# Quaternijkon/hnsw-ivf

Hardware: AMD Instinct MI355X
Metric: queries/sec @ recall@10, IVF4096 d=128 nq=10k nprobe=32; 1/2/4/8 GPUs (higher is better)
Workload: dtype f32; 1 GPU; IVF4096,Flat; d=128, nb=1000000, vectors_per_gpu=1000000, nq_per_gpu=10000, nprobe=32, k=10, global_batch=10000, parallelism=single, grid_point=False

## Files before the change

hnsw-ivf_amd/csrc/bf3.h:

```cpp
#pragma once

#include <hip/hip_runtime.h>

#include <cstdint>

#include "wave_select.h"

namespace faiss_amd {
namespace kern {

typedef __bf16 bf16x8 __attribute__((ext_vector_type(8)));
typedef float floatx16 __attribute__((ext_vector_type(16)));

constexpr int BQ = 64;
constexpr int FQ = 128;
constexpr int BV = 64;
constexpr int BDM = 128;

__device__ __forceinline__ uint32_t med3_u32(uint32_t a, uint32_t b, uint32_t c) {
    uint32_t r;
    asm("v_med3_u32 %0, %1, %2, %3" : "=v"(r) : "v"(a), "v"(b), "v"(c));
    return r;
}

// ... 29 lines not shown
__device__ __forceinline__ float key_decode_lo(uint32_t key, uint32_t lowmask) {
    return L2 ? __uint_as_float(key & ~lowmask) : unordered_f32(key & ~lowmask);
}
template <bool L2>
__device__ __forceinline__ float key_decode_hi(uint32_t key, uint32_t lowmask) {
    return L2 ? __uint_as_float(key | lowmask) : unordered_f32(key | lowmask);
}

__device__ __forceinline__ uint32_t fold_key_bits(float acc) { return __float_as_uint(acc); }
__device__ __forceinline__ void mfma_read_guard() {
    __builtin_amdgcn_sched_barrier(0);
    asm volatile("s_nop 15" ::: "memory");
    __builtin_amdgcn_sched_barrier(0);
}
__device__ __forceinline__ float fold_decode_lo(uint32_t key, uint32_t lowmask) {
    return fmaxf(-2.f * __uint_as_float(key & ~lowmask), 0.f);
}
__device__ __forceinline__ float fold_decode_hi(uint32_t key, uint32_t lowmask) {
    return fmaxf(-2.f * __uint_as_float(key | lowmask), 0.f);
}
template <bool L2>
__device__ __forceinline__ float ivf_decode_lo(uint32_t key, uint32_t lowmask, bool fold) {
    return (L2 && fold) ? fold_decode_lo(key, lowmask) : key_decode_lo<L2>(key, lowmask);
}
template <bool L2>
__device__ __forceinline__ float ivf_decode_hi(uint32_t key, uint32_t lowmask, bool fold) {
    return (L2 && fold) ? fold_decode_hi(key, lowmask) : key_decode_hi<L2>(key, lowmask);
}
__device__ __forceinline__ void split3_bf16(float v, __bf16& h, __bf16& m, __bf16& l) {
    h = (__bf16)v;
    const float r1 = v - (float)h;
    m = (__bf16)r1;
    l = (__bf16)(r1 - (float)m);
}

__device__ __forceinline__ void split8(const float (&v)[8], bf16x8& h, bf16x8& l) {
#pragma unroll
    for (int j = 0; j < 8; j++) {
        const __bf16 hb = (__bf16)v[j];
        h[j] = hb;
        l[j] = (__bf16)(v[j] - (float)hb);
    }
}

template <int NS>
__device__ __forceinline__ void query_raw_load(const float* __restrict__ x, int ldx, int d, int qr,
                                               int lh, float4 (&raw)[2 * NS]) {
    const float* xr = x + (int64_t)(qr < 0 ? 0 : qr) * ldx;
    const int d4 = (d + 3) & ~3;
#pragma unroll
    for (int s = 0; s < NS; s++)
#pragma unroll
        for (int u = 0; u < 2; u++) {
            const int kk = 16 * s + 8 * lh + 4 * u;
            raw[2 * s + u] = *(const float4*)(xr + min(kk, d4 - 4));
        }
}
template <int NS>
__device__ __forceinline__ void query_frags_from_raw(const float4 (&raw)[2 * NS], int d, int lh,
                                                     bf16x8 (&bh)[NS], bf16x8 (&bl)[NS],
                                                     float& xn) {
    xn = 0.f;
#pragma unroll
    for (int s = 0; s < NS; s++) {
        float v[8] = {raw[2 * s].x,     raw[2 * s].y,     raw[2 * s].z,     raw[2 * s].w,
                      raw[2 * s + 1].x, raw[2 * s + 1].y, raw[2 * s + 1].z, raw[2 * s + 1].w};
#pragma unroll
        for (int j = 0; j < 8; j++) v[j] = 16 * s + 8 * lh + j < d ? v[j] : 0.f;
        split8(v, bh[s], bl[s]);
#pragma unroll
        for (int j = 0; j < 8; j++) xn = fmaf(v[j], v[j], xn);
    }
    xn += __shfl_xor(xn, 32);
}
template <int NS>
__device__ __forceinline__ void load_query_frags(const float* __restrict__ x, int ldx, int d,
                                                 int qr, int lh, bf16x8 (&bh)[NS],
                                                 bf16x8 (&bl)[NS], float& xn) {
    float4 raw[2 * NS];
    query_raw_load<NS>(x, ldx, d, qr, lh, raw);
    query_frags_from_raw<NS>(raw, d, lh, bh, bl, xn);
}

template <int NS>
__device__ __forceinline__ void load_query_image(const uint8_t* __restrict__ qimg,
                                                 const float* __restrict__ qxn, int qr, int lh,
                                                 bf16x8 (&bh)[NS], bf16x8 (&bl)[NS], float& xn) {
    const int q = qr < 0 ? 0 : qr;
    const uint8_t* row = qimg + (int64_t)q * (64 * NS) + 16 * lh;
#pragma unroll
    for (int s = 0; s < NS; s++) {
        bh[s] = *(const bf16x8*)(row + 32 * s);
        bl[s] = *(const bf16x8*)(row + 32 * NS + 32 * s);
    }
    xn = qxn ? qxn[q] : 0.f;
}

template <int NS>
__device__ __forceinline__ floatx16 bf3_block(const uint8_t* arow, const bf16x8 (&bh)[NS],
                                              const bf16x8 (&bl)[NS]) {
    constexpr int DB = 16 * NS;
    bf16x8 ah[NS], al[NS];
#pragma unroll
    for (int s = 0; s < NS; s++) {
        ah[s] = *(const bf16x8*)(arow + 32 * s);
        al[s] = *(const bf16x8*)(arow + 2 * DB + 32 * s);
    }
    floatx16 acc;
#pragma unroll
    for (int r = 0; r < 16; r++) acc[r] = 0.f;
#pragma unroll
    for (int s = 0; s < NS; s++) {
        acc = __builtin_amdgcn_mfma_f32_32x32x16_bf16(al[s], bh[s], acc, 0, 0, 0);
        acc = __builtin_amdgcn_mfma_f32_32x32x16_bf16(ah[s], bl[s], acc, 0, 0, 0);
        acc = __builtin_amdgcn_mfma_f32_32x32x16_bf16(ah[s], bh[s], acc, 0, 0, 0);
    }
    return acc;
}

template <int NS>
__device__ __forceinline__ floatx16 bf2_block(const uint8_t* arow, const bf16x8 (&bh)[NS],
                                              const bf16x8 (&bl)[NS]) {
    bf16x8 ah[NS];
#pragma unroll
    for (int s = 0; s < NS; s++) ah[s] = *(const bf16x8*)(arow + 32 * s);
    floatx16 acc;
#pragma unroll
    for (int r = 0; r < 16; r++) acc[r] = 0.f;
#pragma unroll
    for (int s = 0; s < NS; s++) {
        acc = __builtin_amdgcn_mfma_f32_32x32x16_bf16(ah[s], bl[s], acc, 0, 0, 0);
        acc = __builtin_amdgcn_mfma_f32_32x32x16_bf16(ah[s], bh[s], acc, 0, 0, 0);
    }
    return acc;
}

__device__ __forceinline__ uint32_t cdiv_dev(uint32_t a, uint32_t b) { return (a + b - 1) / b; }

__device__ __forceinline__ uint32_t ivf_key_row(uint32_t key, uint32_t lowmask, int slot) {
    const uint32_t ord = key & lowmask;
    const uint32_t r = ord & 15u;
    return (ord >> 4) * BV + 32 * (slot >> 1) + 4 * (slot & 1) + 8 * (r >> 2) + (r & 3);
}

__device__ __forceinline__ int ivf_stream_row(int e, int slot) {
    const int r = e & 15;
    return (e >> 4) * BV + 32 * (slot >> 1) + 4 * (slot & 1) + 8 * (r >> 2) + (r & 3);
}

inline int bf3_db(int d) { return (d + 31) / 32 * 32; }

}
}
```

hnsw-ivf_amd/csrc/core.cpp:

```cpp
#include <algorithm>
#include <cfloat>
#include <cmath>
#include <cstdlib>
#include <cstring>
#include <thread>

#include "../../include/faiss_amd.h"
#include "kernels.h"

namespace faiss_amd {
namespace kern {
void mask_columns(float* D, int64_t nx, int64_t ny, int64_t ldD, const uint8_t* mask, float v,
                  hipStream_t s);
}

IndexIVFStats indexIVF_stats;
HNSWStats hnsw_stats;
HNSWRowStats hnsw_row_stats;

std::mutex InterruptCallback::lock;
std::unique_ptr<InterruptCallback> InterruptCallback::instance;

void InterruptCallback::clear_instance() { instance.reset(); }

// ... 222 lines not shown
            kern::row_resnorm_bf16(d_xb_.as<float>(), ntotal, d, l, s_tile_.as<float>(), s);
            kern::array_max(s_tile_.as<float>(), ntotal, d_cnmax_.as<float>() + 1, s);
            d_cst_.reserve(kern::coarse_stream_image_bytes(ntotal, d));
            const char* fenv = getenv("FAISS_AMD_COARSE_FOLD");
            cfold_ = (metric_type == METRIC_L2 && !(fenv && !strcmp(fenv, "0"))) ? 1 : 0;
            kern::coarse_stream_image(d_xb_.as<float>(), ntotal, d, l, d_norms_.as<float>(),
                                      d_cst_.ptr, s, cfold_);
        }
    }
    HIP_CHECK(hipStreamSynchronize(s));
    dirty_ = false;
}

const float* IndexFlat::device_vectors() const {
    sync_device();
    return d_xb_.as<float>();
}
size_t IndexFlat::query_image_size(idx_t n) const {
    return kern::query_image_bytes(n, d) + sizeof(float) * n;
}
const float* IndexFlat::device_norms() const {
    sync_device();
    return d_norms_.as<float>();
}

template <class OutIdx>
bool IndexFlat::knn_device(idx_t n, const float* x, int ldx, int k, float* distances,
                           OutIdx* labels, hipStream_t s, void* qimg_out, idx_t batch_n) const {
    FAISS_THROW_IF_NOT_FMT(k >= 1, "k = %d must be >= 1", k);
    sync_device();
    std::lock_guard<std::recursive_mutex> g(mu_);
    order_.enter(s);
    const bool direct = (batch_n >= 0 ? batch_n : n) < 20;
    const bool img = knn_impl<OutIdx>(n, x, ldx, k, distances, labels, s, qimg_out, direct);
    order_.leave(s);
    return img;
}

template <class OutIdx>
bool IndexFlat::knn_impl(idx_t n, const float* x, int ldx, int k, float* distances,
                         OutIdx* labels, hipStream_t s, void* qimg_out, bool direct) const {
    const int l = ld();
    const int metric_l2 = metric_type == METRIC_L2;
    const bool ip_chunked = !metric_l2 && ntotal > ((idx_t)1 << 20);
    FAISS_THROW_IF_NOT_MSG(!(ip_chunked && k <= kern::kMaxK && sizeof(OutIdx) == 4),
                           "coarse quantizer larger than 2^20 centroids");
    if (k > kern::kMaxK || ip_chunked) {
        if (metric_l2) {
            s_xn_.reserve(sizeof(float) * std::max<idx_t>(n, 1));
            kern::row_norms(x, n, d, ldx, s_xn_.as<float>(), s);
        }
        const idx_t ny = std::max<idx_t>(ntotal, 1);
        const idx_t qc = std::max<idx_t>(1, std::min<idx_t>(n, ((idx_t)1 << 28) / ny));
        s_tile_.reserve(sizeof(float) * qc * ny);
        ScopedKernelTimer tm(&ktimes, "flat_distance+select_exact", 2.0 * n * ntotal * d, s);
        for (idx_t q0 = 0; q0 < n; q0 += qc) {
            const idx_t nq = std::min(qc, n - q0);
            if (ntotal > 0 && direct)
                kern::direct_distances(x + q0 * ldx, nq, ldx, d_xb_.as<float>(), ntotal, l, d,
                                       metric_l2, s_tile_.as<float>(), ntotal, s);
            else if (ntotal > 0)
                kern::pairwise_distances(x + q0 * ldx, nq, ldx,
                                         metric_l2 ? s_xn_.as<float>() + q0 : nullptr,
                                         d_xb_.as<float>(), ntotal, l, d_norms_.as<float>(), l,
                                         metric_l2, s_tile_.as<float>(), ntotal, s);
            kern::select_rows_exact<OutIdx>(s_tile_.as<float>(), nq, ntotal, ntotal, k,
                                            metric_l2, 0, distances + q0 * k, labels + q0 * k, k,
                                            s, &s_sel_);
        }
        return false;
    }
    constexpr bool i32 = sizeof(OutIdx) == 4;
    int32_t* o32 = i32 ? (int32_t*)labels : nullptr;
    int64_t* o64 = i32 ? nullptr : (int64_t*)labels;
    const idx_t ny = ntotal;
    s_xn_.reserve(sizeof(float) * std::max<idx_t>(n, 1));
    const char* cenv = getenv("FAISS_AMD_COARSE");
    const kern::CoarsePlan plan =
            (cenv && !strcmp(cenv, "f32")) || ny > (1 << 20) || d_cbf_.ptr == nullptr || direct
                    ? kern::CoarsePlan{}
                    : kern::coarse_bf3_plan(n, (int)ny, d, k);
    if (plan.ok) {
        const bool qi = d_cst_.ptr != nullptr && ldx % 4 == 0;
        void* qimg = nullptr;
        if (qi) {
            const size_t ib = kern::query_image_bytes(n, d);
            if (!qimg_out) s_qimg_.reserve(ib + sizeof(float) * n);
            qimg = qimg_out ? qimg_out : s_qimg_.ptr;
            ScopedKernelTimer tq(&ktimes, "query_prep", 0.0, s);
            kern::query_prep(x, n, ldx, d, s_xn_.as<float>(), qimg, (float*)((uint8_t*)qimg + ib),
                             s);
        } else {
            kern::row_norms(x, n, d, ldx, s_xn_.as<float>(), s);
        }
        const size_t per_q = (size_t)plan.entries * 4 + plan.nsplit * 16;
        const idx_t qchunk = std::max<idx_t>(64, (idx_t)(((size_t)256 << 20) / per_q) / 64 * 64);
        const idx_t qc = std::min<idx_t>(qchunk, n);
        s_cand_i_.reserve(sizeof(uint32_t) * qc * plan.entries);
        s_tile_.reserve(sizeof(float) * qc * plan.nsplit * 4);
        for (idx_t q0 = 0; q0 < n; q0 += qc) {
            const idx_t nq = std::min(qc, n - q0);
            kern::coarse_bf3_knn(plan, x + q0 * ldx, nq, ldx, s_xn_.as<float>() + q0,
                                 d_xb_.as<float>(), l, d_cbf_.ptr, d_norms_.as<float>(),
                                 d_cnmax_.as<float>(), (int)ny, d, k, metric_l2,
                                 s_cand_i_.as<uint32_t>(), s_tile_.as<float>(), distances + q0 * k,
                                 o32 ? o32 + q0 * k : nullptr, o64 ? o64 + q0 * k : nullptr, s,
                                 d_cst_.ptr,
                                 qi ? (const uint8_t*)qimg + q0 * kern::query_image_bytes(1, d)
                                    : nullptr,
                                 &ktimes, cfold_);
        }
        return qi && qimg_out;
    }
    if (metric_l2) kern::row_norms(x, n, d, ldx, s_xn_.as<float>(), s);
    const idx_t Yc = std::min<idx_t>(std::max<idx_t>(ny, 1), 1 << 20);
    const idx_t nyc = (idx_t)cdiv(std::max<idx_t>(ny, 1), Yc);
    FAISS_THROW_IF_NOT_MSG(!(i32 && nyc > 1), "coarse quantizer larger than 2^20 centroids");
    const size_t tile_budget = (size_t)256 << 20;
    idx_t qchunk = std::max<idx_t>(128, (idx_t)(tile_budget / (sizeof(float) * Yc)) / 128 * 128);
    qchunk = std::min<idx_t>(qchunk, n);
    s_tile_.reserve(sizeof(float) * qchunk * Yc);
    if (nyc > 1) {
        s_cand_d_.reserve(sizeof(float) * nyc * qchunk * k);
        s_cand_i_.reserve(sizeof(idx_t) * nyc * qchunk * k);
    }
    double flops = 2.0 * (double)n * (double)ny * (double)d;
    ScopedKernelTimer tm(&ktimes, "flat_distance+select", flops, s);
    for (idx_t q0 = 0; q0 < n; q0 += qchunk) {
        const idx_t nq = std::min(qchunk, n - q0);
        const float* xq = x + q0 * ldx;
        const float* xn = s_xn_.as<float>() + q0;
        if (nyc == 1) {
            if (ny > 0 && direct)
                kern::direct_distances(xq, nq, ldx, d_xb_.as<float>(), ny, l, d, metric_l2,
                                       s_tile_.as<float>(), ny, s);
            else if (ny > 0)
                kern::pairwise_distances(xq, nq, ldx, xn, d_xb_.as<float>(), ny, l,
                                         d_norms_.as<float>(), l, metric_l2,
                                         s_tile_.as<float>(), ny, s);
            kern::select_rows(s_tile_.as<float>(), nq, ny, ny, k, metric_l2, 0,
                              distances + q0 * k, o32 ? o32 + q0 * k : nullptr,
                              o64 ? o64 + q0 * k : nullptr, k, s);
            if (!metric_l2 && ny > 0)
                kern::select_fix_ip(s_tile_.as<float>(), nq, ny, ny, k, distances + q0 * k,
                                    o32 ? o32 + q0 * k : nullptr, o64 ? o64 + q0 * k : nullptr,
                                    k, s);
        } else {
            for (idx_t c = 0; c < nyc; c++) {
                const idx_t y0 = c * Yc, nyy = std::min(Yc, ny - y0);
                if (direct)
                    kern::direct_distances(xq, nq, ldx, d_xb_.as<float>() + y0 * l, nyy, l, d,
                                           metric_l2, s_tile_.as<float>(), nyy, s);
                else
                    kern::pairwise_distances(xq, nq, ldx, xn, d_xb_.as<float>() + y0 * l, nyy,
                                             l, d_norms_.as<float>() + y0, l, metric_l2,
                                             s_tile_.as<float>(), nyy, s);
                kern::select_rows(s_tile_.as<float>(), nq, nyy, nyy, k, metric_l2, y0,
                                  s_cand_d_.as<float>() + c * nq * k, nullptr,
                                  s_cand_i_.as<int64_t>() + c * nq * k, k, s);
            }
            kern::merge_rows(s_cand_d_.as<float>(), s_cand_i_.as<int64_t>(), nq,
                             (int)((nyc << 16) | k), k, metric_l2, distances + q0 * k,
                             o64 + q0 * k, s);
        }
    }
    return false;
}

void IndexFlat::search_device(idx_t n, const float* x, int ldx, idx_t k, float* distances,
                              idx_t* labels, const SearchParameters* params,
                              hipStream_t s) const {
    DeviceGuard g(device);
    if (params && params->sel) {
        search_selected(n, x, ldx, k, distances, labels, params->sel, s);
        return;
    }
    knn_device<idx_t>(n, x, ldx, (int)k, distances, labels, s);
}

const idx_t* IndexFlat::device_row_ids(hipStream_t s) const {
    std::lock_guard<std::recursive_mutex> g(mu_);
    if (selids_n_ != ntotal) {
        std::vector<idx_t> iota((size_t)ntotal);
        for (idx_t i = 0; i < ntotal; i++) iota[(size_t)i] = i;
        s_selids_.reserve(sizeof(idx_t) * ntotal);
        HIP_CHECK(hipMemcpyAsync(s_selids_.ptr, iota.data(), sizeof(idx_t) * ntotal,
                                 hipMemcpyHostToDevice, s));
        HIP_CHECK(hipStreamSynchronize(s));
        selids_n_ = ntotal;
    }
    return s_selids_.as<idx_t>();
}

// ... 366 lines not shown
```

hnsw-ivf_amd/csrc/kernels.h:

```cpp
#pragma once

#include <hip/hip_runtime.h>
#include <algorithm>
#include <cstdint>

#include "common.h"

namespace faiss_amd {
namespace kern {

constexpr int kMaxK = 64;
constexpr int kMaxNprobeFilter = 2048;
constexpr int kMaxKExact = 2048;

void row_norms(const float* x, int64_t n, int d, int ld, float* out, hipStream_t s);

void pairwise_distances(const float* x, int64_t nx, int ldx, const float* xn,
                        const float* y, int64_t ny, int ldy, const float* yn, int dp,
                        int metric_l2, float* D, int64_t ldD, hipStream_t s);

void direct_distances(const float* x, int64_t nx, int ldx, const float* y, int64_t ny, int ldy,
                      int d, int metric_l2, float* D, int64_t ldD, hipStream_t s);

struct CoarsePlan {
    bool ok = false;
    int nsplit = 0, split_len = 0, kt = 0, obits = 0, entries = 0;
};
CoarsePlan coarse_bf3_plan(int64_t n, int nlist, int d, int k);
void coarse_bf3_knn(const CoarsePlan& p, const float* x, int64_t n, int ldx, const float* xnorm,
                    const float* cent, int ldc, const void* cbf, const float* cnorm,
                    const float* cnmax, int nlist, int d, int k, int metric_l2, uint32_t* keys,
                    float* pbs, float* D, int32_t* I32, int64_t* I64, hipStream_t s,
                    const void* cst = nullptr, const void* qimg = nullptr,
                    KernelTimes* kt = nullptr,
                    int fold = 0);
void query_prep(const float* x, int64_t n, int ldx, int d, float* ref_norms, void* qimg,
                float* qxn, hipStream_t s);
inline size_t query_image_bytes(int64_t n, int d) {
    return (size_t)std::max<int64_t>(n, 1) * 4 * ((d + 31) / 32 * 32);
}
void coarse_stream_image(const float* codes, int64_t rows, int d, int ldc, const float* norms,
                         void* out, hipStream_t s, int fold = 0);
size_t coarse_stream_image_bytes(int64_t rows, int d);
void array_max(const float* a, int64_t n, float* out, hipStream_t s);

void select_rows(const float* D, int64_t nx, int64_t ny, int64_t ldD, int k, int metric_l2,
                 int64_t col0, float* out_d, int32_t* out_i32, int64_t* out_i64,
                 int64_t ldo, hipStream_t s);

void select_fix_ip(const float* D, int64_t nx, int64_t ny, int64_t ldD, int k, float* out_d,
                   int32_t* out_i32, int64_t* out_i64, int64_t ldo, hipStream_t s);

void merge_rows(const float* cand_d, const int64_t* cand_i, int64_t n, int nin_x_kin, int k,
                int metric_l2, float* out_d, int64_t* out_i, hipStream_t s);

void merge_rows_general(const float* cand_d, const int64_t* cand_i, int64_t n, int nshard,
                        int kin, int k, int metric_l2, float* out_d, int64_t* out_i,
                        hipStream_t s);

void translate_labels(int64_t* labels, int64_t n, int64_t offset, hipStream_t s);

struct alignas(16) ProbeRec {
    float pb[4];
    float mmax;
    uint32_t off;
    uint32_t len;
    uint32_t pad;
};

struct alignas(16) ItemDesc {
    uint32_t l, nq, len, off;
};

struct IVFBuckets {
    uint32_t* counts;
    uint32_t* bucket_off;
    uint32_t* item_off;
    uint32_t* cursor;
    uint32_t* entries;
    uint32_t* item_list = nullptr;
    uint32_t* item_ctr = nullptr;
    uint32_t* scan_tmp = nullptr;
    uint32_t* ticket = nullptr;
    const uint32_t* perm = nullptr;
    ItemDesc* item_desc = nullptr;
    uint32_t* item_entries = nullptr;
    uint32_t* mark_keys = nullptr;
    ProbeRec* mark_recs = nullptr;
    int mark_ke = 0;
    uint32_t* counts_next = nullptr;
    const uint32_t* lim = nullptr;
    const uint8_t* sel = nullptr;
};
void probe_limits(const int32_t* assign, int64_t n, int nprobe, const uint32_t* list_len,
                  int nlist, int64_t max_codes, int32_t* assign_out, uint32_t* lim,
                  hipStream_t s);
void ivf_bucket(const int32_t* assign, int64_t n, int nprobe, const uint32_t* list_len,
                const uint32_t* list_off, int nlist, int QT, IVFBuckets b, hipStream_t s);
void ivf_flat_rerank(const uint32_t* keys, const ProbeRec* recs, const float* x, int ldx,
                     const float* codes, int ldc, const int64_t* ids, int d, int64_t n,
                     int nprobe, int KE, int obits, int k, int metric_l2, const uint8_t* sel,
                     uint32_t* stats, float* D, int64_t* I, KernelTimes* kt, hipStream_t s,
                     unsigned long long* qdone, int fold);
struct PQArgs {
    const float* pq_cent = nullptr;
    const float* cent = nullptr;
    int ldcent = 0;
    const float* cdis = nullptr;
    const uint8_t* codes = nullptr;
    int cs = 0;
    int M = 0;
    int table1 = 0;
};
struct RerankSel {
    const uint8_t* sel = nullptr;
};
bool ivfpq_mfma_eligible(int d, int M, int k, int nprobe);
double ivfpq_mfma_coef(int d, int M);
// ... 238 lines not shown
```

hnsw-ivf_amd/csrc/kernels_coarse.hip:

```cpp
#include <hip/hip_runtime.h>

#include <algorithm>
#include <cfloat>
#include <cstdio>
#include <cstdlib>
#include <cstring>
#include <type_traits>
#include <vector>

#include "bf3.h"
#include "common.h"
#include "exact_select.h"
#include "kernels.h"
#include "ref_arith.h"
#include "wave_select.h"

namespace faiss_amd {
namespace kern {

__device__ __forceinline__ float ip_seq(const float* __restrict__ a, const float* __restrict__ b,
                                        int d) {
    float acc = 0.f;
    int j = 0;
    for (; j + 32 <= d; j += 32) {
// ... 59 lines not shown
#pragma unroll
        for (int s = 0; s < PF; s++) {
            const int e = t + 256 * s;
            const int r = e / RU, c = e - r * RU;
            pf[s] = make_uint4(0u, 0u, 0u, 0u);
            if (e < BV * RU && r < nvn)
                pf[s] = *(const uint4*)(cbf + (int64_t)(c0 + v0n + r) * (2 * DB) + 8 * c);
        }
        if (t < BV / 4) {
            const int r = 4 * t;
            float v[4];
#pragma unroll
            for (int c = 0; c < 4; c++)
                v[c] = r + c < nvn ? (L2 ? cn[v0n + r + c] : 0.f) : WS_INF;
            pn = make_float4(v[0], v[1], v[2], v[3]);
        }
    };
    auto stash = [&](int buf) {
        uint8_t* T = tiles + buf * BV * CSB;
#pragma unroll
        for (int s = 0; s < PF; s++) {
            const int e = t + 256 * s;
            const int r = e / RU, c = e - r * RU;
            if (e < BV * RU) *(uint4*)(T + r * CSB + 16 * c) = pf[s];
        }
        if (t < BV / 4) *(float4*)(&ynt[buf][4 * t]) = pn;
    };
    fetch(0);
    stash(0);
    if (BV < len) fetch(BV);
    __syncthreads();

    ThreadQueue32<KT> tq;
    tq.init();
    const uint32_t lowmask = (1u << obits) - 1u;
    for (int v0 = 0, tile = 0; v0 < len; v0 += BV, tile++) {
        const int buf = tile & 1;
        if (v0 + BV < len) {
            stash(buf ^ 1);
            if (v0 + 2 * BV < len) fetch(v0 + 2 * BV);
        }
        float4 yq[4];
#pragma unroll
        for (int g = 0; g < 4; g++) yq[g] = *(const float4*)(&ynt[buf][32 * bi + 4 * lh + 8 * g]);
        const uint8_t* arow = tiles + buf * BV * CSB + (32 * bi + li) * CSB + 16 * lh;
        const floatx16 acc = Y3 ? bf3_block<NS>(arow, bh, bl) : bf2_block<NS>(arow, bh, bl);
        const uint32_t ordbase = (uint32_t)tile << 4;
#pragma unroll
        for (int r = 0; r < 16; r++) {
            const int g = r >> 2, c = r & 3;
            const float yv = c == 0 ? yq[g].x : c == 1 ? yq[g].y : c == 2 ? yq[g].z : yq[g].w;
            const float a = L2 ? fmaf(-2.f, acc[r], xn + yv) : yv - acc[r];
            tq.push(key_encode<L2>(a, lowmask, ordbase | (uint32_t)r));
        }
        __syncthreads();
    }
    if (q < n) {
        const float M = coarse_margin(xn, cnmax_p, coef, Y3);
        const int E1 = 4 * KT;
        uint32_t* ko = keys + (q * nsplit + sp) * E1 + slot * KT;
#pragma unroll
        for (int i = 0; i < KT; i++) {
            const uint32_t key = tq.q[i];
            const uint32_t row = ivf_key_row(key, lowmask, slot);
            ko[i] = (key != 0xffffffffu && row < (uint32_t)len) ? key : 0xffffffffu;
        }
        const uint32_t last = tq.q[KT - 1];
        float bnd = WS_INF;
        if (last != 0xffffffffu && ivf_key_row(last, lowmask, slot) < (uint32_t)len)
            bnd = key_decode_lo<L2>(last, lowmask);
        pbs[(q * nsplit + sp) * 4 + slot] = bnd < WS_INF ? bnd - M : WS_INF;
    }
}

template <int N>
__device__ __forceinline__ void cwait_vmcnt() {
    static_assert(N >= 0 && N < 64, "vmcnt range");
    __builtin_amdgcn_s_waitcnt((N & 15) | (7 << 4) | (15 << 8) | ((N >> 4) << 14));
}

template <bool L2, int KT, int NS, bool FOLD = false>
__global__ __launch_bounds__(256, NS <= 6 && KT <= 8 ? 3 : 2) void k_coarse_stream(
        const float* __restrict__ x, int ldx, int64_t n, int d, const uint8_t* __restrict__ cst,
        const float* __restrict__ xnorm, int nlist, int nsplit, int split_len, int nqb,
        float coef, const float* __restrict__ cnmax_p, int obits, uint32_t* __restrict__ keys,
        float* __restrict__ pbs, unsigned long long* __restrict__ trace,
        const uint8_t* __restrict__ qimg) {
    unsigned long long* tr = (trace && threadIdx.x == 0) ? trace + 160ull * blockIdx.x : nullptr;
    if (tr) tr[0] = __builtin_amdgcn_s_memtime();
    constexpr int DB = 16 * NS;
    constexpr int SR = 4 * DB + 16;
    constexpr int TB = BV * SR;
    static_assert(TB % 1024 == 0, "tile = whole 1 KB glds blocks");
    constexpr int NG = TB / 1024;
    constexpr int G0 = (NG + 3) / 4;
    constexpr int G3 = NG / 4;
    __shared__ __attribute__((aligned(16))) uint8_t tiles[2 * TB];
    const int t = threadIdx.x, lane = t & 63, w = t >> 6;
    const int li = lane & 31, lh = lane >> 5;
    int sp, qb;
    if ((nsplit & 7) == 0) {
        const int xcd = blockIdx.x & 7, m = blockIdx.x >> 3;
        sp = 8 * (m / nqb) + xcd;
        qb = m % nqb;
    } else {
        sp = blockIdx.x / nqb;
        qb = blockIdx.x % nqb;
    }
    const int c0 = sp * split_len;
    const int len = min(split_len, nlist - c0);
    const int ntile = (len + BV - 1) / BV;
    const int qloc = 32 * w + li;
    const int64_t q = (int64_t)qb * 128 + qloc;
    const bool active = (int64_t)qb * 128 + 32 * w < n;

    auto issue = [&](int j, int b) {
        const uint8_t* src = cst + ((int64_t)c0 + (int64_t)j * BV) * SR + 16 * lane;
        uint8_t* dst = tiles + b * TB;
#pragma unroll
        for (int g = 0; g < G0; g++) {
            const int blk = w + 4 * g;
            if (g < G3 || blk < NG)
                __builtin_amdgcn_global_load_lds(
                        (const void*)(src + blk * 1024),
                        (__attribute__((address_space(3))) void*)(dst + blk * 1024), 16, 0, 0);
        }
    };
    issue(0, 0);
    bf16x8 bh[NS], bl[NS];
    float xn_approx;
    if (active) {
        if (qimg)
            load_query_image<NS>(qimg, nullptr, q < n ? (int)q : -1, lh, bh, bl, xn_approx);
        else
            load_query_frags<NS>(x, ldx, d, q < n ? (int)q : -1, lh, bh, bl, xn_approx);
    }
    const float xn = (active && q < n) ? xnorm[q] : 0.f;
    if (tr) tr[1] = __builtin_amdgcn_s_memtime();
    static_assert(!FOLD || L2, "fold: L2 only");
    bf16x8 bq;
    if constexpr (FOLD) {
        __bf16 h, m, lo;
        split3_bf16(-0.5f * xn, h, m, lo);
        const __bf16 one = (__bf16)1.f, zero = (__bf16)0.f;
        bq[0] = lh ? zero : one;
        bq[1] = lh ? zero : one;
        bq[2] = lh ? zero : one;
        bq[3] = lh ? zero : h;
        bq[4] = lh ? zero : m;
        bq[5] = lh ? zero : lo;
        bq[6] = zero;
        bq[7] = zero;
    }

    ThreadQueue32<KT> tq[2];
    tq[0].init();
    tq[1].init();
    const uint32_t lowmask = (1u << obits) - 1u;
    auto norms = [&](const uint8_t* T, int bi, float (&nv)[16]) {
        const uint8_t* nrow = T + (32 * bi + 4 * lh) * SR + 4 * DB;
#pragma unroll
        for (int r = 0; r < 16; r++) nv[r] = *(const float*)(nrow + (8 * (r >> 2) + (r & 3)) * SR);
    };
    auto push1 = [&](ThreadQueue32<KT>& pq, float accr, float yv0, uint32_t ord) {
        if constexpr (FOLD) {
            pq.push(key_insert(fold_key_bits(accr), lowmask, ord));
            return;
        }
        const float yv = L2 ? yv0 : (yv0 < WS_INF ? 0.f : WS_INF);
        const float a = L2 ? fmaf(-2.f, accr, xn + yv) : yv - accr;
        pq.push(key_insert(key_bits<L2>(a), lowmask, ord));
    };
    auto mfma_push = [&](const uint8_t* T, int bi, const floatx16& pacc, const float (&pn)[16],
                         const uint8_t* pnT, uint32_t pord, ThreadQueue32<KT>& pq) {
        const uint8_t* arow = T + (32 * bi + li) * SR + 16 * lh;
        bf16x8 ah[NS], al[NS];
#pragma unroll
        for (int s2 = 0; s2 < NS; s2++) {
            ah[s2] = *(const bf16x8*)(arow + 32 * s2);
            al[s2] = *(const bf16x8*)(arow + 2 * DB + 32 * s2);
        }
        floatx16 acc;
#pragma unroll
        for (int r = 0; r < 16; r++) acc[r] = 0.f;
#pragma unroll
        for (int s2 = 0; s2 < NS; s2++) {
            acc = __builtin_amdgcn_mfma_f32_32x32x16_bf16(al[s2], bh[s2], acc, 0, 0, 0);
            acc = __builtin_amdgcn_mfma_f32_32x32x16_bf16(ah[s2], bl[s2], acc, 0, 0, 0);
            acc = __builtin_amdgcn_mfma_f32_32x32x16_bf16(ah[s2], bh[s2], acc, 0, 0, 0);
            if (FOLD && s2 == 0) mfma_read_guard();
#pragma unroll
            for (int r = 16 * s2 / NS; r < 16 * (s2 + 1) / NS; r++)
                push1(pq, pacc[r],
                      FOLD ? 0.f
                           : pnT ? *(const float*)(pnT + (8 * (r >> 2) + (r & 3)) * SR) : pn[r],
                      pord | (uint32_t)r);
        }
        if constexpr (FOLD) {
            const bf16x8 ab = *(const bf16x8*)(T + (32 * bi + li) * SR + (lh ? 0 : 4 * DB));
            acc = __builtin_amdgcn_mfma_f32_32x32x16_bf16(ab, bq, acc, 0, 0, 0);
        }
        return acc;
    };
    floatx16 acc0, acc1;
    float n1[16];
    cwait_vmcnt<0>();
    __builtin_amdgcn_s_barrier();
    if (ntile > 1) issue(1, 1);
    if (active) {
        acc0 = bf3_block<NS>(tiles + (0 * SR) + li * SR + 16 * lh, bh, bl);
        if constexpr (FOLD) {
            const bf16x8 ab = *(const bf16x8*)(tiles + li * SR + (lh ? 0 : 4 * DB));
            acc0 = __builtin_amdgcn_mfma_f32_32x32x16_bf16(ab, bq, acc0, 0, 0, 0);
        }
    }
    int b = 0;
    for (int j = 0; j < ntile; j++) {
        const uint8_t* T = tiles + b * TB;
        const uint32_t ordbase = (uint32_t)j << 4;
        if (active) {
// ... 462 lines not shown
        trace[8 * q + 3] = t_u;
        trace[8 * q + 4] = t_c;
        trace[8 * q + 5] = t_e;
        trace[8 * q + 7] = t_f;
    }
    if (stats && valid && lane == 0) {
        atomicAdd(&stats[0], (uint32_t)min(ns, CR_CAP));
        atomicAdd(&stats[1], (uint32_t)__popcll(fmask));
        atomicAdd(&stats[2], st.overflow ? 1u : 0u);
        atomicAdd(&stats[3], done ? 0u : 1u);
        atomicAdd(&stats[4], relayed ? 1u : 0u);
    }
}

__global__ void k_array_max(const float* __restrict__ a, int64_t n, float* __restrict__ out) {
    __shared__ float red[16];
    float m = 0.f;
    for (int64_t i = threadIdx.x; i < n; i += blockDim.x) {
        const float v = a[i];
        m = v < WS_INF ? fmaxf(m, v) : WS_INF;
    }
#pragma unroll
    for (int s = 32; s > 0; s >>= 1) m = fmaxf(m, __shfl_xor(m, s));
    if ((threadIdx.x & 63) == 0) red[threadIdx.x >> 6] = m;
    __syncthreads();
    if (threadIdx.x == 0) {
        float r = 0.f;
        for (int i = 0; i < (int)(blockDim.x >> 6); i++) r = fmaxf(r, red[i]);
        *out = r;
    }
}

CoarsePlan coarse_bf3_plan(int64_t n, int nlist, int d, int k) {
    CoarsePlan p{};
    if (n < 20 || nlist <= 0 || k < 1 || k > kMaxK || bf3_db(d) > BDM)
        return p;
    int ncu = 256, dev = 0;
    if (hipGetDevice(&dev) != hipSuccess ||
        hipDeviceGetAttribute(&ncu, hipDeviceAttributeMultiprocessorCount, dev) != hipSuccess ||
        ncu <= 0)
        ncu = 256;
    (void)hipGetLastError();
    const int64_t nqb = (int64_t)cdiv((size_t)n, 128);

    const bool big_image = coarse_stream_image_bytes(nlist, d) > ((size_t)4 << 20);
    int nsplit = 0, kt = 0, split_len = 0;
    double best = 0.0;
    const char* nsenv = getenv("FAISS_AMD_COARSE_NSPLIT");
    const int ns_force = nsenv ? atoi(nsenv) : 0;
    for (int ns = 1; ns <= std::min(16, std::max(1, nlist / BV)); ns++) {
        if (ns_force > 0 && ns != ns_force) continue;
        if (k > 16 * ns) continue;
        const double lam = (double)k / (4.0 * ns);
        if (lam > 4.0) continue;
        const int kt1 = lam <= 0.25 ? 4 : lam <= 2.0 ? 8 : 16;
        const int sl = (int)roundup(cdiv((size_t)nlist, (size_t)ns), BV);
        const int nsp = (int)cdiv((size_t)nlist, (size_t)sl);
        if ((size_t)sl > ((size_t)BV << 10)) continue;
        const int64_t slots = (bf3_db(d) <= 96 && kt1 <= 8 ? 3 : 2) * (int64_t)ncu;
        const int64_t rounds = (int64_t)cdiv((size_t)(nqb * nsp), (size_t)slots);
        double cost = (double)rounds * (double)cdiv((size_t)sl, BV) * (kt1 + 12);
        if (big_image && nsp % 8 != 0) cost *= 1.15;
        if (nsplit == 0 || cost < best) {
            best = cost;
            nsplit = nsp;
            kt = kt1;
            split_len = sl;
        }
    }
    if (nsplit == 0) return p;
    const int tiles = (int)cdiv((size_t)split_len, BV);
    int b = 0;
    while ((1 << b) < tiles) b++;
    if (4 + b > 14) return p;
    p.ok = true;
    p.nsplit = nsplit;
    p.split_len = split_len;
    p.kt = kt;
    p.obits = 4 + b;
    p.entries = nsplit * 4 * kt;
    return p;
}

void coarse_bf3_knn(const CoarsePlan& p, const float* x, int64_t n, int ldx, const float* xnorm,
                    const float* cent, int ldc, const void* cbf, const float* cnorm,
                    const float* cnmax, int nlist, int d, int k, int metric_l2, uint32_t* keys,
                    float* pbs, float* D, int32_t* I32, int64_t* I64, hipStream_t s,
                    const void* cst, const void* qimg, KernelTimes* kt, int fold) {
    if (n <= 0) return;
    FAISS_THROW_IF_NOT(p.ok);
    static uint32_t* stats = nullptr;
    const bool dbg = getenv("FAISS_AMD_IVF_STATS") != nullptr;
    if (dbg && !stats) HIP_CHECK(hipMalloc(&stats, 32));
    if (dbg) HIP_CHECK(hipMemsetAsync(stats, 0, 32, s));
    FAISS_THROW_IF_NOT(ldx % 4 == 0 && ldc % 4 == 0);
    const int NS = bf3_db(d) / 16;
    const char* prec = getenv("FAISS_AMD_COARSE_PREC");
    const bool y3 = !(prec && !strcmp(prec, "bf16x2"));
    const char* cenv = getenv("FAISS_AMD_COARSE");
    const bool stream = cst && y3 && !(cenv && !strcmp(cenv, "staged"));
    const bool fk = stream && fold != 0 && metric_l2;
    const float coef = (float)(fk ? ivf_bf3f_coef(d) : y3 ? ivf_bf3_coef(d) : ivf_bf2_coef(d));
    static unsigned long long* ctrace_buf = nullptr;
    static int64_t ctrace_n = 0;
    const char* ctr = getenv("FAISS_AMD_COARSE_TRACE");
    unsigned long long* ctrace = nullptr;
    const int64_t nqb = (int64_t)cdiv((size_t)n, stream ? 128 : BQ);
    const int64_t grid = nqb * p.nsplit;
    FAISS_THROW_IF_NOT(grid < (1ll << 31));
    if (ctr && stream) {
        if (ctrace_n < grid) {
            if (ctrace_buf) HIP_CHECK(hipFree(ctrace_buf));
            HIP_CHECK(hipMalloc(&ctrace_buf, 160 * 8 * grid));
            ctrace_n = grid;
        }
        HIP_CHECK(hipMemsetAsync(ctrace_buf, 0, 160 * 8 * grid, s));
        ctrace = ctrace_buf;
    }
#define LAUNCH_NS(L2V, KTV, NSV)                                                              \
    do {                                                                                      \
        if (stream)                                                                           \
            (fk ? k_coarse_stream<L2V, KTV, NSV, L2V> : k_coarse_stream<L2V, KTV, NSV, false>) \
                    <<<kgrid(grid, 256), dim3(256), 0, s>>>(                              \
                    x, ldx, n, d, (const uint8_t*)cst, xnorm, nlist, p.nsplit, p.split_len,   \
                    (int)nqb, coef, cnmax, p.obits, keys, pbs, ctrace,                        \
                    (const uint8_t*)qimg);                                                    \
        else if (y3)                                                                          \
            k_coarse_bf3_filter<L2V, KTV, NSV, true><<<kgrid(grid, 256), dim3(256), 0, s>>>( \
                    x, ldx, n, d, (const __bf16*)cbf, cnorm, xnorm, nlist, p.nsplit,          \
                    p.split_len, coef, cnmax, p.obits, keys, pbs);                            \
        else                                                                                  \
            k_coarse_bf3_filter<L2V, KTV, NSV, false><<<kgrid(grid, 256), dim3(256), 0, s>>>( \
                    x, ldx, n, d, (const __bf16*)cbf, cnorm, xnorm, nlist, p.nsplit,          \
                    p.split_len, coef, cnmax, p.obits, keys, pbs);                            \
    } while (0)
#define LAUNCH_A(L2V, KTV)                     \
    do {                                       \
        if (NS == 2) LAUNCH_NS(L2V, KTV, 2);   \
        else if (NS == 4) LAUNCH_NS(L2V, KTV, 4); \
        else if (NS == 6) LAUNCH_NS(L2V, KTV, 6); \
        else LAUNCH_NS(L2V, KTV, 8);           \
    } while (0)
#define DISPATCH(L2V)                      \
    do {                                   \
        if (p.kt == 4) LAUNCH_A(L2V, 4);   \
        else if (p.kt == 8) LAUNCH_A(L2V, 8); \
        else LAUNCH_A(L2V, 16);            \
    } while (0)
    {
        ScopedKernelTimer tm(kt, "coarse_filter", 0.0, s);
        if (metric_l2) DISPATCH(true);
        else DISPATCH(false);
    }
#undef DISPATCH
#undef LAUNCH_A
#undef LAUNCH_NS
    HIP_LAUNCH_CHECK();
    if (ctrace) {
        std::vector<unsigned long long> h(160 * grid);
        HIP_CHECK(hipMemcpyAsync(h.data(), ctrace, 160 * 8 * grid, hipMemcpyDeviceToHost, s));
        HIP_CHECK(hipStreamSynchronize(s));
        if (FILE* f = fopen(ctr, "wb")) {
            fwrite(h.data(), 8, h.size(), f);
            fclose(f);
        }
    }
    const int E = p.entries;
    const int V = E <= 64 ? 1 : E <= 128 ? 2 : E <= 256 ? 4 : E <= 512 ? 8 : 16;
    FAISS_THROW_IF_NOT(E <= 1024 && V <= p.kt);
#define LAUNCH_R(L2V, OT, OUT, VV)                                                              \
    k_coarse_rerank<L2V, OT, VV><<<kgrid(n, 64), dim3(64), 0, s>>>(                       \
            keys, pbs, x, ldx, xnorm, cent, ldc, cnorm, cnmax, coef, y3 ? 1 : 0, n, d, nlist,  \
            p.nsplit,                                                                           \
            p.split_len, p.kt, p.obits, k, D, OUT, st_ptr, crtrace, fk ? 1 : 0)
#define LAUNCH_RV(L2V, OT, OUT)                  \
    do {                                         \
        if (V == 1) LAUNCH_R(L2V, OT, OUT, 1);   \
        else if (V == 2) LAUNCH_R(L2V, OT, OUT, 2); \
        else if (V == 4) LAUNCH_R(L2V, OT, OUT, 4); \
        else if (V == 8) LAUNCH_R(L2V, OT, OUT, 8); \
        else LAUNCH_R(L2V, OT, OUT, 16);         \
    } while (0)
    uint32_t* const st_ptr = dbg ? stats : nullptr;
    static unsigned long long* crtrace_buf = nullptr;
    static int64_t crtrace_n = 0;
    const char* crt = getenv("FAISS_AMD_CRERANK_TRACE");
    unsigned long long* crtrace = nullptr;
    if (crt) {
        if (crtrace_n < n) {
            if (crtrace_buf) HIP_CHECK(hipFree(crtrace_buf));
            HIP_CHECK(hipMalloc(&crtrace_buf, 64 * n));
            crtrace_n = n;
        }
        HIP_CHECK(hipMemsetAsync(crtrace_buf, 0, 64 * n, s));
        crtrace = crtrace_buf;
    }
    {
        ScopedKernelTimer tm(kt, "coarse_rerank", 0.0, s);
        if (metric_l2) {
            if (I32) LAUNCH_RV(true, int32_t, I32);
            else LAUNCH_RV(true, int64_t, I64);
        } else {
            if (I32) LAUNCH_RV(false, int32_t, I32);
            else LAUNCH_RV(false, int64_t, I64);
        }
    }
#undef LAUNCH_RV
#undef LAUNCH_R
    if (crtrace) {
// ... 27 lines not shown
```

Measured before the change: 40.01 million queries/s.

## Fuse query prep into streaming coarse kernel, writing query image and norms in-kernel

Result: no change. 40.37 million queries/s (median of 6 runs) (+0.9%).

```diff
diff --git a/hnsw-ivf_amd/csrc/bf3.h b/hnsw-ivf_amd/csrc/bf3.h
--- a/hnsw-ivf_amd/csrc/bf3.h
+++ b/hnsw-ivf_amd/csrc/bf3.h
@@ -135,6 +135,57 @@
     query_frags_from_raw<NS>(raw, d, lh, bh, bl, xn);
 }
 
+__device__ __forceinline__ void half_swap(float p, float q, float& a, float& b) {
+    const auto r = __builtin_amdgcn_permlane32_swap(__float_as_uint(p), __float_as_uint(q), false,
+                                                    false);
+    a = __uint_as_float(r[0]);
+    b = __uint_as_float(r[1]);
+}
+
+template <int NS>
+__device__ __forceinline__ void load_query_frags_norm(const float* __restrict__ x, int ldx, int d,
+                                                      int qr, int lh, bf16x8 (&bh)[NS],
+                                                      bf16x8 (&bl)[NS], float& xn, float& rn) {
+    float4 raw[2 * NS];
+    query_raw_load<NS>(x, ldx, d, qr, lh, raw);
+    const int n8 = d & ~7;
+    float c0 = 0.f, c1 = 0.f, c2 = 0.f, c3 = 0.f;
+#pragma unroll
+    for (int s = 0; s < NS; s++) {
+        float4 a, b;
+        half_swap(raw[2 * s].x, raw[2 * s + 1].x, a.x, b.x);
+        half_swap(raw[2 * s].y, raw[2 * s + 1].y, a.y, b.y);
+        half_swap(raw[2 * s].z, raw[2 * s + 1].z, a.z, b.z);
+        half_swap(raw[2 * s].w, raw[2 * s + 1].w, a.w, b.w);
+        if (16 * s + 8 > n8) a = make_float4(0.f, 0.f, 0.f, 0.f);
+        if (16 * s + 16 > n8) b = make_float4(0.f, 0.f, 0.f, 0.f);
+        c0 = fmaf(a.x, a.x, c0);
+        c1 = fmaf(a.y, a.y, c1);
+        c2 = fmaf(a.z, a.z, c2);
+        c3 = fmaf(a.w, a.w, c3);
+        c0 = fmaf(b.x, b.x, c0);
+        c1 = fmaf(b.y, b.y, c1);
+        c2 = fmaf(b.z, b.z, c2);
+        c3 = fmaf(b.w, b.w, c3);
+    }
+    const float x0 = c0 + __shfl_xor(c0, 32), x1 = c1 + __shfl_xor(c1, 32);
+    const float x2 = c2 + __shfl_xor(c2, 32), x3 = c3 + __shfl_xor(c3, 32);
+    float r = (x0 + x2) + (x1 + x3);
+    if (n8 < d) {
+        const float* a = x + (int64_t)(qr < 0 ? 0 : qr) * ldx;
+        int i = n8;
+        if (d - n8 >= 4) {
+            const float4 av = *(const float4*)(a + n8);
+            const float e0 = av.x * av.x, e1 = av.y * av.y, e2 = av.z * av.z, e3 = av.w * av.w;
+            r = r + ((e0 + e2) + (e1 + e3));
+            i += 4;
+        }
+        for (; i < d; i++) r = fmaf(a[i], a[i], r);
+    }
+    rn = r;
+    query_frags_from_raw<NS>(raw, d, lh, bh, bl, xn);
+}
+
 template <int NS>
 __device__ __forceinline__ void load_query_image(const uint8_t* __restrict__ qimg,
                                                  const float* __restrict__ qxn, int qr, int lh,
diff --git a/hnsw-ivf_amd/csrc/core.cpp b/hnsw-ivf_amd/csrc/core.cpp
--- a/hnsw-ivf_amd/csrc/core.cpp
+++ b/hnsw-ivf_amd/csrc/core.cpp
@@ -328,15 +328,18 @@
                     : kern::coarse_bf3_plan(n, (int)ny, d, k);
     if (plan.ok) {
         const bool qi = d_cst_.ptr != nullptr && ldx % 4 == 0;
+        const bool fused = qi && kern::coarse_bf3_streams(d_cst_.ptr);
         void* qimg = nullptr;
+        const size_t ib = kern::query_image_bytes(n, d);
         if (qi) {
-            const size_t ib = kern::query_image_bytes(n, d);
             if (!qimg_out) s_qimg_.reserve(ib + sizeof(float) * n);
             qimg = qimg_out ? qimg_out : s_qimg_.ptr;
+        }
+        if (qi && !fused) {
             ScopedKernelTimer tq(&ktimes, "query_prep", 0.0, s);
             kern::query_prep(x, n, ldx, d, s_xn_.as<float>(), qimg, (float*)((uint8_t*)qimg + ib),
                              s);
-        } else {
+        } else if (!qi) {
             kern::row_norms(x, n, d, ldx, s_xn_.as<float>(), s);
         }
         const size_t per_q = (size_t)plan.entries * 4 + plan.nsplit * 16;
@@ -352,9 +355,9 @@
                                  s_cand_i_.as<uint32_t>(), s_tile_.as<float>(), distances + q0 * k,
                                  o32 ? o32 + q0 * k : nullptr, o64 ? o64 + q0 * k : nullptr, s,
                                  d_cst_.ptr,
-                                 qi ? (const uint8_t*)qimg + q0 * kern::query_image_bytes(1, d)
-                                    : nullptr,
-                                 &ktimes, cfold_);
+                                 qi ? (uint8_t*)qimg + q0 * kern::query_image_bytes(1, d) : nullptr,
+                                 &ktimes, cfold_,
+                                 fused ? (float*)((uint8_t*)qimg + ib) + q0 : nullptr);
         }
         return qi && qimg_out;
     }
diff --git a/hnsw-ivf_amd/csrc/kernels.h b/hnsw-ivf_amd/csrc/kernels.h
--- a/hnsw-ivf_amd/csrc/kernels.h
+++ b/hnsw-ivf_amd/csrc/kernels.h
@@ -27,13 +27,14 @@
     int nsplit = 0, split_len = 0, kt = 0, obits = 0, entries = 0;
 };
 CoarsePlan coarse_bf3_plan(int64_t n, int nlist, int d, int k);
-void coarse_bf3_knn(const CoarsePlan& p, const float* x, int64_t n, int ldx, const float* xnorm,
+void coarse_bf3_knn(const CoarsePlan& p, const float* x, int64_t n, int ldx, float* xnorm,
                     const float* cent, int ldc, const void* cbf, const float* cnorm,
                     const float* cnmax, int nlist, int d, int k, int metric_l2, uint32_t* keys,
                     float* pbs, float* D, int32_t* I32, int64_t* I64, hipStream_t s,
-                    const void* cst = nullptr, const void* qimg = nullptr,
-                    KernelTimes* kt = nullptr,
-                    int fold = 0);
+                    const void* cst = nullptr, void* qimg = nullptr, KernelTimes* kt = nullptr,
+                    int fold = 0,
+                    float* qxn = nullptr);
+bool coarse_bf3_streams(const void* cst);
 void query_prep(const float* x, int64_t n, int ldx, int d, float* ref_norms, void* qimg,
                 float* qxn, hipStream_t s);
 inline size_t query_image_bytes(int64_t n, int d) {
diff --git a/hnsw-ivf_amd/csrc/kernels_coarse.hip b/hnsw-ivf_amd/csrc/kernels_coarse.hip
--- a/hnsw-ivf_amd/csrc/kernels_coarse.hip
+++ b/hnsw-ivf_amd/csrc/kernels_coarse.hip
@@ -165,10 +165,10 @@
 template <bool L2, int KT, int NS, bool FOLD = false>
 __global__ __launch_bounds__(256, NS <= 6 && KT <= 8 ? 3 : 2) void k_coarse_stream(
         const float* __restrict__ x, int ldx, int64_t n, int d, const uint8_t* __restrict__ cst,
-        const float* __restrict__ xnorm, int nlist, int nsplit, int split_len, int nqb,
-        float coef, const float* __restrict__ cnmax_p, int obits, uint32_t* __restrict__ keys,
-        float* __restrict__ pbs, unsigned long long* __restrict__ trace,
-        const uint8_t* __restrict__ qimg) {
+        float* xnorm, int nlist, int nsplit, int split_len, int nqb, float coef,
+        const float* __restrict__ cnmax_p, int obits, uint32_t* __restrict__ keys,
+        float* __restrict__ pbs, unsigned long long* __restrict__ trace, uint8_t* qimg,
+        float* qxn) {
     unsigned long long* tr = (trace && threadIdx.x == 0) ? trace + 160ull * blockIdx.x : nullptr;
     if (tr) tr[0] = __builtin_amdgcn_s_memtime();
     constexpr int DB = 16 * NS;
@@ -212,13 +212,33 @@
     issue(0, 0);
     bf16x8 bh[NS], bl[NS];
     float xn_approx;
+    float xn = 0.f;
     if (active) {
-        if (qimg)
-            load_query_image<NS>(qimg, nullptr, q < n ? (int)q : -1, lh, bh, bl, xn_approx);
-        else
-            load_query_frags<NS>(x, ldx, d, q < n ? (int)q : -1, lh, bh, bl, xn_approx);
-    }
-    const float xn = (active && q < n) ? xnorm[q] : 0.f;
+        const int qr = q < n ? (int)q : -1;
+        if (qxn) {
+            float rn;
+            load_query_frags_norm<NS>(x, ldx, d, qr, lh, bh, bl, xn_approx, rn);
+            if (qr >= 0) xn = rn;
+            if (sp == 0 && qr >= 0) {
+                uint8_t* row = qimg + q * (64 * NS) + 16 * lh;
+#pragma unroll
+                for (int s2 = 0; s2 < NS; s2++) {
+                    *(bf16x8*)(row + 32 * s2) = bh[s2];
+                    *(bf16x8*)(row + 32 * NS + 32 * s2) = bl[s2];
+                }
+                if (lh == 0) {
+                    qxn[q] = xn_approx;
+                    xnorm[q] = rn;
+                }
+            }
+        } else {
+            if (qimg)
+                load_query_image<NS>(qimg, nullptr, qr, lh, bh, bl, xn_approx);
+            else
+                load_query_frags<NS>(x, ldx, d, qr, lh, bh, bl, xn_approx);
+            if (qr >= 0) xn = xnorm[q];
+        }
+    }
     if (tr) tr[1] = __builtin_amdgcn_s_memtime();
     static_assert(!FOLD || L2, "fold: L2 only");
     bf16x8 bq;
@@ -847,11 +867,17 @@
     return p;
 }
 
-void coarse_bf3_knn(const CoarsePlan& p, const float* x, int64_t n, int ldx, const float* xnorm,
+bool coarse_bf3_streams(const void* cst) {
+    const char* prec = getenv("FAISS_AMD_COARSE_PREC");
+    const char* cenv = getenv("FAISS_AMD_COARSE");
+    return cst && !(prec && !strcmp(prec, "bf16x2")) && !(cenv && !strcmp(cenv, "staged"));
+}
+
+void coarse_bf3_knn(const CoarsePlan& p, const float* x, int64_t n, int ldx, float* xnorm,
                     const float* cent, int ldc, const void* cbf, const float* cnorm,
                     const float* cnmax, int nlist, int d, int k, int metric_l2, uint32_t* keys,
                     float* pbs, float* D, int32_t* I32, int64_t* I64, hipStream_t s,
-                    const void* cst, const void* qimg, KernelTimes* kt, int fold) {
+                    const void* cst, void* qimg, KernelTimes* kt, int fold, float* qxn) {
     if (n <= 0) return;
     FAISS_THROW_IF_NOT(p.ok);
     static uint32_t* stats = nullptr;
@@ -862,8 +888,8 @@
     const int NS = bf3_db(d) / 16;
     const char* prec = getenv("FAISS_AMD_COARSE_PREC");
     const bool y3 = !(prec && !strcmp(prec, "bf16x2"));
-    const char* cenv = getenv("FAISS_AMD_COARSE");
-    const bool stream = cst && y3 && !(cenv && !strcmp(cenv, "staged"));
+    FAISS_THROW_IF_NOT(!qxn || (cst && qimg));
+    const bool stream = qxn ? true : coarse_bf3_streams(cst);
     const bool fk = stream && fold != 0 && metric_l2;
     const float coef = (float)(fk ? ivf_bf3f_coef(d) : y3 ? ivf_bf3_coef(d) : ivf_bf2_coef(d));
     static unsigned long long* ctrace_buf = nullptr;
@@ -888,8 +914,7 @@
             (fk ? k_coarse_stream<L2V, KTV, NSV, L2V> : k_coarse_stream<L2V, KTV, NSV, false>) \
                     <<<kgrid(grid, 256), dim3(256), 0, s>>>(                              \
                     x, ldx, n, d, (const uint8_t*)cst, xnorm, nlist, p.nsplit, p.split_len,   \
-                    (int)nqb, coef, cnmax, p.obits, keys, pbs, ctrace,                        \
-                    (const uint8_t*)qimg);                                                    \
+                    (int)nqb, coef, cnmax, p.obits, keys, pbs, ctrace, (uint8_t*)qimg, qxn);  \
         else if (y3)                                                                          \
             k_coarse_bf3_filter<L2V, KTV, NSV, true><<<kgrid(grid, 256), dim3(256), 0, s>>>( \
                     x, ldx, n, d, (const __bf16*)cbf, cnorm, xnorm, nlist, p.nsplit,          \
```
